# auniquesun/PPT

Measured on AMD Instinct MI355X. Metric: point-clouds/sec fwd+bwd, PointBERT 1024-pt ModelNet40, higher is better.
Workload: dtype f16; 1 GPU; C2: ModelNet40 1024-pt PointBERT (ULIP_PointBERT head_type=0, frozen backbone + PromptLearner), train-mode BN + DropPath, fwd + CE(ls 0.2) + bwd + AdamW; feed=resident, per_gpu_batch=32, global_batch=32, npoints=1024, classes=40, parallelism=dp1

## Files before the change

### ppt_amd/csrc/attention.hip

```cpp
#include "attn_common.h"

namespace {

constexpr int SEG = 16, KT = 32, ROWS = 64;

__device__ __forceinline__ float quad_sum(float v)
{
    v += __uint_as_float(dpp_mov<0xB1, 0xf>(__float_as_uint(v)));
    v += __uint_as_float(dpp_mov<0x4E, 0xf>(__float_as_uint(v)));
    return v;
}

template <typename T>
__device__ __forceinline__ void stage_rows(const T *__restrict__ base, int64_t row_stride, int r0, int Tlen,
                                           float *dst, int Tfull, int P, int v)
{
    for (int i = threadIdx.x; i < KT * HD; i += blockDim.x) {
        const int r = i >> 6, d = i & 63;
        dst[i] = (r0 + r) < Tlen ? dt<T>::load(base + am_row(Tfull, P, v, r0 + r) * row_stride + d) : 0.0f;
    }
}

template <typename T>
__global__ __launch_bounds__(256) void attn_fwd_quad(const T *__restrict__ qkv, T *__restrict__ out,
// ... 167 lines not shown
        dk[d] = 0.f; dv[d] = 0.f;
    }
    const int nqt = (Tlen + KT - 1) / KT;
    const int qt0 = causal ? (blockIdx.x * ROWS) / KT : 0;
    for (int qt = qt0; qt < nqt; ++qt) {
        __syncthreads();
        stage_rows<T>(qb, rs, qt * KT, Tlen, Qs, Tfull, P, b);
        stage_rows<T>(gb, (int64_t)H * HD, qt * KT, Tlen, Gs, Tfull, P, b);
        if (threadIdx.x < KT) {
            const int qi = qt * KT + threadIdx.x;
            Ls[threadIdx.x] = qi < Tlen ? lse[am_stat(Tfull, P, H, b, h, qi)] : 0.f;
            Ds[threadIdx.x] = qi < Tlen ? delta[am_stat(Tfull, P, H, b, h, qi)] : 0.f;
        }
        __syncthreads();
#pragma unroll 4
        for (int i = 0; i < KT; ++i) {
            float s = 0.f, dp = 0.f;
#pragma unroll
            for (int d = 0; d < SEG; ++d) {
                s = fmaf(Qs[i * HD + seg * SEG + d], k[d], s);
                dp = fmaf(Gs[i * HD + seg * SEG + d], v[d], dp);
            }
            s = quad_sum(s) * scale;
            dp = quad_sum(dp);
            const int qi = qt * KT + i;
            const bool ok = active && qi < Tlen && qi >= q_lo && (!causal || kj <= qi);
            const float p = ok ? __expf(s - Ls[i]) : 0.f;
            const float ds = p * (dp - Ds[i]) * scale;
#pragma unroll
            for (int d = 0; d < SEG; ++d) {
                dv[d] = fmaf(p, Gs[i * HD + seg * SEG + d], dv[d]);
                dk[d] = fmaf(ds, Qs[i * HD + seg * SEG + d], dk[d]);
            }
        }
    }
    if (active && P > 0 && kj < P) {
        float *pk = part + (((int64_t)b * P + kj) * 2) * (H * HD) + h * HD + seg * SEG, *pv = pk + H * HD;
#pragma unroll
        for (int d = 0; d < SEG; ++d) { pk[d] = dk[d]; pv[d] = dv[d]; }
    } else if (active) {
        T *o = dqkv + am_row(Tfull, P, b, kj) * rs + h * HD + seg * SEG;
#pragma unroll
        for (int d = 0; d < SEG; ++d) {
            dt<T>::store(o + H * HD + d, dk[d]);
            dt<T>::store(o + 2 * H * HD + d, dv[d]);
        }
    }
}

template <typename T>
__global__ __launch_bounds__(256) void attn_prefix_reduce(const float *__restrict__ part, int nseq, int P, int HHD, T *__restrict__ dqkv, int prio)
{
    PPT_PRIO(prio);
    const int i = blockIdx.x * 256 + threadIdx.x;
    if (i >= P * 2 * HHD) return;
    float acc = 0.f;
    const float *src = part + i;
    const int64_t stride = (int64_t)P * 2 * HHD;
    int v = 0;
    for (; v + 8 <= nseq; v += 8) {
        float t[8];
#pragma unroll
        for (int u = 0; u < 8; ++u) t[u] = src[(v + u) * stride];
#pragma unroll
        for (int u = 0; u < 8; ++u) acc += t[u];
    }
    for (; v < nseq; ++v) acc += src[v * stride];
    const int pos = i / (2 * HHD), rem = i - pos * 2 * HHD;
    dt<T>::store(dqkv + (int64_t)pos * 3 * HHD + HHD + rem, acc);
}

template <typename T>
int attn_fwd_t(const void *qkv, void *out, float *lse, int Bt, int Tl, int H, float scale, int causal, int P, hipStream_t s)
{
    dim3 grid((Tl + ROWS - 1) / ROWS, (Bt + (P > 0)) * H);
    hipLaunchKernelGGL(attn_fwd_quad<T>, grid, dim3(256), 0, s, (const T *)qkv, (T *)out, lse, Tl, H, scale, causal, P, Bt);
    PPT_CHECK_LAUNCH();
    return PPT_OK;
}

__host__ int64_t attn_rows(int Bt, int Tl, int P) { return P > 0 ? (int64_t)P + (int64_t)Bt * (Tl - P) : (int64_t)Bt * Tl; }

template <typename T>
int attn_reduce_t(const float *part, void *dqkv, int Bt, int P, int H, int prio, hipStream_t s)
{
    if (P <= 0) return PPT_OK;
    const int n = P * 2 * H * HD;
    hipLaunchKernelGGL(attn_prefix_reduce<T>, dim3((n + 255) / 256), dim3(256), 0, s, part, Bt + 1, P, H * HD, (T *)dqkv, prio);
    PPT_CHECK_LAUNCH();
    return PPT_OK;
}

template <typename T>
int attn_bwd_t(const void *qkv, const void *out, const void *dout, const float *lse, float *delta, void *dqkv,
               int Bt, int Tl, int H, float scale, int causal, int P, float *part, bool with_delta, hipStream_t s)
{
    if (with_delta) {
        const int64_t rows = attn_rows(Bt, Tl, P) * H;
        hipLaunchKernelGGL(attn_delta<T>, dim3((unsigned)((rows + 63) / 64)), dim3(256), 0, s, (const T *)out,
                           (const T *)dout, delta, Tl, H, rows, P);
        PPT_CHECK_LAUNCH();
    }
    dim3 grid((Tl + ROWS - 1) / ROWS, (Bt + (P > 0)) * H);
    hipLaunchKernelGGL(attn_bwd_dq<T>, grid, dim3(256), 0, s, (const T *)qkv, (const T *)dout, lse, delta, (T *)dqkv,
                       Tl, H, scale, causal, P, Bt);
    PPT_CHECK_LAUNCH();
    hipLaunchKernelGGL(attn_bwd_dkv<T>, grid, dim3(256), 0, s, (const T *)qkv, (const T *)dout, lse, delta, (T *)dqkv,
                       Tl, H, scale, causal, P, Bt, part);
    PPT_CHECK_LAUNCH();
    return attn_reduce_t<T>(part, dqkv, Bt, P, H, ppt_get_wave_priority(), s);
}

}

static int attn_fwd_any(const void *qkv, void *out, float *lse, int Bt, int T, int P, int H, int hd, float scale, int causal,
                        int dtype, void *stream)
{
    if (!qkv || !out || Bt <= 0 || T <= 0 || H <= 0 || hd != HD) return PPT_EINVAL;
    if (dtype == PPT_F32) return attn_fwd_t<float>(qkv, out, lse, Bt, T, H, scale, causal, P, ppt_stream(stream));
    if (dtype == PPT_BF16 || dtype == PPT_F16) return ppt_attention_fwd_mfma_bf16(qkv, out, lse, Bt, T, H, scale, causal, P, dtype, ppt_stream(stream));
    return PPT_EINVAL;
}

extern "C" int ppt_attention_fwd(const void *qkv, void *out, float *lse, int Bt, int T, int H, int hd, float scale,
                                 int causal, int dtype, void *stream)
{
    return attn_fwd_any(qkv, out, lse, Bt, T, 0, H, hd, scale, causal, dtype, stream);
}

extern "C" int ppt_attention_fwd_quad_bf16(const void *qkv, void *out, float *lse, int Bt, int T, int H, float scale,
                                           int causal, int P, int fmt, hipStream_t s)
{
    return fmt == PPT_F16 ? attn_fwd_t<f16_t>(qkv, out, lse, Bt, T, H, scale, causal, P, s) : attn_fwd_t<bf16_t>(qkv, out, lse, Bt, T, H, scale, causal, P, s);
}

extern "C" int ppt_attention_prefix_reduce_f32(const float *part, void *dqkv, int Bt, int P, int H, int prio, hipStream_t s)
{
    return attn_reduce_t<float>(part, dqkv, Bt, P, H, prio, s);
}

static int attn_bwd_any(const void *qkv, const void *out, const void *dout, const float *lse, float *delta, void *dqkv, float *part,
                        int Bt, int T, int P, int H, int hd, float scale, int causal, int dtype, void *stream)
{
    if (!qkv || !out || !dout || !lse || !delta || !dqkv || Bt <= 0 || T <= 0 || H <= 0 || hd != HD) return PPT_EINVAL;
    if (P > 0 && !part) return PPT_EINVAL;
    if (dtype == PPT_F32)
        return attn_bwd_t<float>(qkv, out, dout, lse, delta, dqkv, Bt, T, H, scale, causal, P, part, true, ppt_stream(stream));
    if (dtype == PPT_BF16 || dtype == PPT_F16) {
        hipStream_t s = ppt_stream(stream);
        const bool f16 = dtype == PPT_F16;
        const int prio = ppt_get_wave_priority();
        auto reduce = [&]() { return f16 ? attn_reduce_t<f16_t>(part, dqkv, Bt, P, H, prio, s) : attn_reduce_t<bf16_t>(part, dqkv, Bt, P, H, prio, s); };
        if (T <= 128) {
            const int rc = ppt_attention_bwd_short_mfma_bf16(qkv, out, dout, lse, dqkv, Bt, T, H, scale, causal, P, part, dtype, s);
            if (rc == PPT_OK) return reduce();
            if (rc != PPT_EUNSUPPORTED) return rc;
        }
        const int64_t rows = attn_rows(Bt, T, P) * H;
        if (f16)
            hipLaunchKernelGGL(attn_delta<f16_t>, dim3((unsigned)((rows + 63) / 64)), dim3(256), 0, s, (const f16_t *)out,
                               (const f16_t *)dout, delta, T, H, rows, P);
        else
            hipLaunchKernelGGL(attn_delta<bf16_t>, dim3((unsigned)((rows + 63) / 64)), dim3(256), 0, s, (const bf16_t *)out,
                               (const bf16_t *)dout, delta, T, H, rows, P);
        PPT_CHECK_LAUNCH();
        const int rc = ppt_attention_bwd_mfma_bf16(qkv, dout, lse, delta, dqkv, Bt, T, H, scale, causal, P, part, dtype, s);
        if (rc == PPT_OK) return reduce();
        if (rc != PPT_EUNSUPPORTED) return rc;
        return f16 ? attn_bwd_t<f16_t>(qkv, out, dout, lse, delta, dqkv, Bt, T, H, scale, causal, P, part, false, s)
                   : attn_bwd_t<bf16_t>(qkv, out, dout, lse, delta, dqkv, Bt, T, H, scale, causal, P, part, false, s);
    }
    return PPT_EINVAL;
}

extern "C" int ppt_attention_bwd(const void *qkv, const void *out, const void *dout, const float *lse, float *delta,
                                 void *dqkv, int Bt, int T, int H, int hd, float scale, int causal, int dtype,
                                 void *stream)
{
    return attn_bwd_any(qkv, out, dout, lse, delta, dqkv, nullptr, Bt, T, 0, H, hd, scale, causal, dtype, stream);
}

extern "C" size_t ppt_attention_prefix_workspace_bytes(int C, int P, int H, int hd)
{
    return (size_t)(C + 1) * (size_t)P * 2 * (size_t)H * (size_t)hd * sizeof(float);
}

extern "C" int ppt_attention_prefix_fwd(const void *qkv, void *out, float *lse, int C, int T, int P, int H, int hd, float scale,
                                        int dtype, void *stream)
{
    if (P <= 0 || P >= T) return PPT_EINVAL;
    return attn_fwd_any(qkv, out, lse, C, T, P, H, hd, scale, 1, dtype, stream);
}

extern "C" int ppt_attention_prefix_bwd(const void *qkv, const void *out, const void *dout, const float *lse, float *delta,
                                        void *dqkv, float *part, int C, int T, int P, int H, int hd, float scale, int dtype,
                                        void *stream)
{
    if (P <= 0 || P >= T) return PPT_EINVAL;
    return attn_bwd_any(qkv, out, dout, lse, delta, dqkv, part, C, T, P, H, hd, scale, 1, dtype, stream);
}
```

### ppt_amd/csrc/attention_mfma.hip

```cpp
#include <stdlib.h>
#include <type_traits>
#include "attn_bwd16.h"

namespace {

template <int FORM> struct AttnForm {
    using F = typename std::conditional<FORM == PPT_BF16, bf16_t, f16_t>::type;
    using T = bf16_t;
    using chunk_t = uint4;
    static constexpr int IMAGES = 1, CH_SHIFT = 3;
    static constexpr float P_PRE = 1.0f;
    struct Q { chunk_t raw[4][1]; };

    static __device__ __forceinline__ chunk_t zero() { return make_uint4(0, 0, 0, 0); }
    static __device__ __forceinline__ void prep_q(Q &, int) {}
    static __device__ __forceinline__ void write(unsigned char *kimg, unsigned char *vimg, int row, int ch, const chunk_t &k, const chunk_t &v)
    {
        *reinterpret_cast<uint4 *>(kimg + k_off(row, ch)) = k;
        *reinterpret_cast<uint4 *>(vimg + v_off(row, ch * 16)) = v;
    }
    static __device__ __forceinline__ float peel_dot(const T *kl, const Q &q, int h)
    {
        float dot = 0.f;
#pragma unroll
// ... 648 lines not shown
            const float *DL = reinterpret_cast<const float *>(base + 4 * QTILE + 128);
            ATTN_BWD_DKV_STEP(base + 0 * QTILE, base + 1 * QTILE, base + 2 * QTILE, base + 3 * QTILE, L2, DL, 0, qt * QT);
        }
        if (qt + 1 < nqt) write_tile(cur ^ 1);
        __syncthreads();
    }
    if (key < T && P > 0 && key < P) {
        float *pk = part + (((int64_t)b * P + key) * 2) * os + head * HD;
        attn_store_dkdv_part(pk, pk + os, dkt, dvt, h);
    } else if (key < T) {
        bf16_t *ok = dqkv + am_row(Tfull, P, b, key) * rs + head * HD + H * HD;
        attn_store_dkdv16<F>(ok, ok + H * HD, dkt, dvt, h);
    }
}

template <bool CAUSAL, typename F>
__global__ __launch_bounds__(256, 2) void attn_bwd_dkv_mfma(const bf16_t *__restrict__ qkv, const bf16_t *__restrict__ dout,
                                                         const float *__restrict__ lse, const float *__restrict__ delta,
                                                         bf16_t *__restrict__ dqkv, int Tfull, int H, float scale, int P, int C,
                                                         float *__restrict__ part)
{
    __shared__ __align__(16) unsigned char smem[DKV_SMEM];
    attn_bwd_dkv_body<F, CAUSAL, false>(qkv, nullptr, dout, lse, delta, dqkv, Tfull, H, scale, P, C, part, smem, blockIdx.x, blockIdx.y);
}

constexpr int DQ_SMEM = 2 * 3 * TILE;

template <typename F, bool CAUSAL, bool INLINE_DELTA>
__device__ __forceinline__ void attn_bwd_dq_body(const bf16_t *__restrict__ qkv, const bf16_t *__restrict__ out, const bf16_t *__restrict__ dout,
                                                 const float *__restrict__ lse, const float *__restrict__ delta,
                                                 bf16_t *__restrict__ dqkv, int Tfull, int H, float scale, int P, int C,
                                                 unsigned char *smem, const int bx, const int by)
{
    const int lane = threadIdx.x & 63;
    const int w = __builtin_amdgcn_readfirstlane(threadIdx.x >> 6);
    const int r = lane & 31, h = lane >> 5;
    const int bh = by, b = bh / H, head = bh % H;
    const int64_t rs = 3 * (int64_t)H * HD, os = (int64_t)H * HD;
    const int T = am_len(Tfull, P, C, b), q_lo = am_qlo(P, C, b);
    const bf16_t *qb = qkv + head * HD;
    const bf16_t *kb = qb + H * HD, *vb = qb + 2 * H * HD;
    const bf16_t *gb = dout + head * HD;
    const int q0 = bx * QB + w * 32;
    const int qrow = q0 + r;
    const float c = scale * 1.4426950408889634f;

    uint4 qf[4], gf[4];
    float dsum = 0.f;
#pragma unroll
    for (int kk = 0; kk < 4; ++kk) {
        uint4 a = make_uint4(0, 0, 0, 0), v = make_uint4(0, 0, 0, 0);
        if (qrow < T) {
            a = *reinterpret_cast<const uint4 *>(qb + am_row(Tfull, P, b, qrow) * rs + 16 * kk + 8 * h);
            v = *reinterpret_cast<const uint4 *>(gb + am_row(Tfull, P, b, qrow) * os + 16 * kk + 8 * h);
            if constexpr (INLINE_DELTA)
                dsum += dot8_bf16<F>(v, *reinterpret_cast<const uint4 *>(out + head * HD + am_row(Tfull, P, b, qrow) * os + 16 * kk + 8 * h));
        }
        qf[kk] = (a);
        gf[kk] = (v);
    }
    const bool own = qrow < T && qrow >= q_lo;
    const float l2 = own ? lse[am_stat(Tfull, P, H, b, head, qrow)] * 1.4426950408889634f : INFINITY;
    float dl;
    if constexpr (INLINE_DELTA) {
        const float ds = xor32_sum(dsum);
        dl = own ? ds : 0.f;
    } else dl = own ? delta[am_stat(Tfull, P, H, b, head, qrow)] : 0.f;

    uint4 sk[2], sv[2];
    auto load_tile = [&](int kt) {
#pragma unroll
        for (int i = 0; i < 2; ++i) {
            const int cidx = threadIdx.x + 256 * i;
            const int kx = kt * KVT + (cidx >> 3), ch = cidx & 7;
            sk[i] = sv[i] = make_uint4(0, 0, 0, 0);
            if (kx < T) {
                const int64_t kr = am_row(Tfull, P, b, kx) * rs;
                sk[i] = *reinterpret_cast<const uint4 *>(kb + kr + ch * 8);
                sv[i] = *reinterpret_cast<const uint4 *>(vb + kr + ch * 8);
            }
        }
    };
    auto write_tile = [&](int buf) {
#pragma unroll
        for (int i = 0; i < 2; ++i) {
            const int cidx = threadIdx.x + 256 * i;
            const int row = cidx >> 3, ch = cidx & 7;
            unsigned char *base = smem + buf * 3 * TILE;
            *reinterpret_cast<uint4 *>(base + 0 * TILE + k_off(row, ch)) = sk[i];
            *reinterpret_cast<uint4 *>(base + 1 * TILE + v_off(row, ch * 16)) = sk[i];
            *reinterpret_cast<uint4 *>(base + 2 * TILE + k_off(row, ch)) = sv[i];
        }
    };
    const int q_hi = min(T, (int)(bx + 1) * QB) - 1;
    const int nkt = CAUSAL ? min((T + KVT - 1) / KVT, q_hi / KVT + 1) : (T + KVT - 1) / KVT;
    f32x16_t dqt[2];
    ATTN_ZERO2(dqt[0], dqt[1]);
    int tr_row, tr_dbyte;
    tr_lane(lane, tr_row, tr_dbyte);

    load_tile(0);
    write_tile(0);
    __syncthreads();
    for (int kt = 0; kt < nkt; ++kt) {
        const int cur = kt & 1;
        if (kt + 1 < nkt) load_tile(kt + 1);
        const bool active = q0 < T && (!CAUSAL || kt * KVT <= q0 + 31);
        if (active) {
            const unsigned char *base = smem + cur * 3 * TILE;
            const bool need_mask = (kt * KVT + KVT > T) || (CAUSAL && kt * KVT + KVT - 1 > q0);
#pragma unroll
            for (int sub = 0; sub < 2; ++sub)
                ATTN_BWD_DQ_STEP(base + 0 * TILE, base + 1 * TILE, base + 2 * TILE, 32 * sub, kt * KVT + 32 * sub, need_mask);
        }
        if (kt + 1 < nkt) write_tile(cur ^ 1);
        __syncthreads();
    }
    if (own) attn_store_dq16<F>(dqkv + am_row(Tfull, P, b, qrow) * rs + head * HD, dqt, h);
}

template <bool CAUSAL, typename F>
__global__ __launch_bounds__(256, 2) void attn_bwd_dq_mfma(const bf16_t *__restrict__ qkv, const bf16_t *__restrict__ dout,
                                                        const float *__restrict__ lse, const float *__restrict__ delta,
                                                        bf16_t *__restrict__ dqkv, int Tfull, int H, float scale, int P, int C)
{
    __shared__ __align__(16) unsigned char smem[DQ_SMEM];
    attn_bwd_dq_body<F, CAUSAL, false>(qkv, nullptr, dout, lse, delta, dqkv, Tfull, H, scale, P, C, smem, blockIdx.x, blockIdx.y);
}

#ifndef PPT_SHORT_OCC
#define PPT_SHORT_OCC 2
#endif
template <bool CAUSAL, typename F>
__global__ __launch_bounds__(256, PPT_SHORT_OCC) void attn_bwd_short_mfma(const bf16_t *__restrict__ qkv, const bf16_t *__restrict__ out,
                                                           const bf16_t *__restrict__ dout, const float *__restrict__ lse,
                                                           bf16_t *__restrict__ dqkv, int Tfull, int H, float scale, int P, int C,
                                                           float *__restrict__ part, int prio)
{
    PPT_PRIO(prio);
    __shared__ __align__(16) unsigned char smem[DQ_SMEM > DKV_SMEM ? DQ_SMEM : DKV_SMEM];
#ifdef PPT_SHORT_ROLE
    if (PPT_SHORT_ROLE == 0) { attn_bwd_dkv_body<F, CAUSAL, true>(qkv, out, dout, lse, nullptr, dqkv, Tfull, H, scale, P, C, part, smem, 0, blockIdx.y); return; }
    if (PPT_SHORT_ROLE == 1) { attn_bwd_dq_body<F, CAUSAL, true>(qkv, out, dout, lse, nullptr, dqkv, Tfull, H, scale, P, C, smem, 0, blockIdx.y); return; }
    if (PPT_SHORT_ROLE == 2) return;
#endif
    if (gridDim.x == 1 || blockIdx.x == 0)
        attn_bwd_dkv_body<F, CAUSAL, true>(qkv, out, dout, lse, nullptr, dqkv, Tfull, H, scale, P, C, part, smem, 0, blockIdx.y);
    if (gridDim.x == 1) __syncthreads();
    if (gridDim.x == 1 || blockIdx.x == 1)
        attn_bwd_dq_body<F, CAUSAL, true>(qkv, out, dout, lse, nullptr, dqkv, Tfull, H, scale, P, C, smem, 0, blockIdx.y);
}


constexpr int TINY_SMEM = 7 * TILE + 512;
template <bool CAUSAL, typename F>
__global__ __launch_bounds__(256, 2) void attn_bwd_tiny_mfma(const bf16_t *__restrict__ qkv, const bf16_t *__restrict__ out,
                                                          const bf16_t *__restrict__ dout, const float *__restrict__ lse,
                                                          bf16_t *__restrict__ dqkv, int Tfull, int H, float scale, int P, int C,
                                                          float *__restrict__ part, int prio)
{
    PPT_PRIO(prio);
    __shared__ __align__(16) unsigned char smem[TINY_SMEM];
    unsigned char *Qr = smem, *Qt = smem + TILE, *Gr = smem + 2 * TILE, *Gt = smem + 3 * TILE, *Kr = smem + 4 * TILE, *Kt = smem + 5 * TILE,
                  *Vr = smem + 6 * TILE;
    float *L2 = reinterpret_cast<float *>(smem + 7 * TILE), *DL = L2 + 64;
    const int lane = threadIdx.x & 63;
    const int w = __builtin_amdgcn_readfirstlane(threadIdx.x >> 6);
    const int r = lane & 31, h = lane >> 5;
    const int bh = blockIdx.y, b = bh / H, head = bh % H;
    const int64_t rs = 3 * (int64_t)H * HD, os = (int64_t)H * HD;
    const int T = am_len(Tfull, P, C, b), q_lo = am_qlo(P, C, b);
    const float c = scale * 1.4426950408889634f;

    {
        uint4 q[2], k[2], v[2], g[2];
        float dl[2], l2[2];
#pragma unroll
        for (int i = 0; i < 2; ++i) {
            const int row = 32 * i + (threadIdx.x >> 3), ch = threadIdx.x & 7;
            q[i] = k[i] = v[i] = g[i] = make_uint4(0, 0, 0, 0);
            uint4 o = make_uint4(0, 0, 0, 0);
            l2[i] = INFINITY;
            const bool own = row < T && row >= q_lo;
            if (row < T) {
                const int64_t pr = am_row(Tfull, P, b, row);
                const bf16_t *qp = qkv + pr * rs + head * HD + ch * 8;
                q[i] = *reinterpret_cast<const uint4 *>(qp);
                k[i] = *reinterpret_cast<const uint4 *>(qp + H * HD);
                v[i] = *reinterpret_cast<const uint4 *>(qp + 2 * H * HD);
                g[i] = *reinterpret_cast<const uint4 *>(dout + pr * os + head * HD + ch * 8);
                o = *reinterpret_cast<const uint4 *>(out + pr * os + head * HD + ch * 8);
                if (own && ch == 0) l2[i] = lse[am_stat(Tfull, P, H, b, head, row)] * 1.4426950408889634f;
            }
            float d = dot8_bf16<F>(g[i], o);
            d += __shfl_xor(d, 1); d += __shfl_xor(d, 2); d += __shfl_xor(d, 4);
            dl[i] = own ? d : 0.f;
        }
#pragma unroll
        for (int i = 0; i < 2; ++i) {
            const int row = 32 * i + (threadIdx.x >> 3), ch = threadIdx.x & 7;
            *reinterpret_cast<uint4 *>(Qr + k_off(row, ch)) = q[i];
            *reinterpret_cast<uint4 *>(Qt + v_off(row, ch * 16)) = q[i];
            *reinterpret_cast<uint4 *>(Gr + k_off(row, ch)) = g[i];
            *reinterpret_cast<uint4 *>(Gt + v_off(row, ch * 16)) = g[i];
            *reinterpret_cast<uint4 *>(Kr + k_off(row, ch)) = k[i];
            *reinterpret_cast<uint4 *>(Kt + v_off(row, ch * 16)) = k[i];
            *reinterpret_cast<uint4 *>(Vr + k_off(row, ch)) = v[i];
            if (ch == 0) { L2[row] = l2[i]; DL[row] = dl[i]; }
        }
    }
    __syncthreads();
    int tr_row, tr_dbyte;
    tr_lane(lane, tr_row, tr_dbyte);

    if (w < 2) {
        const int k0 = 32 * w, key = k0 + r;
        if (k0 >= T) return;
        uint4 kf[4], vf[4];
#pragma unroll
        for (int kk = 0; kk < 4; ++kk) {
            kf[kk] = *reinterpret_cast<const uint4 *>(Kr + k_off(key, 2 * kk + h));
            vf[kk] = *reinterpret_cast<const uint4 *>(Vr + k_off(key, 2 * kk + h));
        }
        f32x16_t dvt[2], dkt[2];
#pragma unroll
    for (int i = 0; i < 2; ++i) ATTN_ZERO2(dvt[i], dkt[i]);
        const int nqt = (T + QT - 1) / QT;
        for (int qt = q_lo / QT; qt < nqt; ++qt) {
            if (CAUSAL && qt * QT + QT - 1 < k0) continue;
            ATTN_BWD_DKV_STEP(Qr, Qt, Gr, Gt, L2, DL, QT * qt, qt * QT);
        }
        if (key < T && P > 0 && key < P) {
            float *pk = part + (((int64_t)b * P + key) * 2) * os + head * HD;
            attn_store_dkdv_part(pk, pk + os, dkt, dvt, h);
        } else if (key < T) {
            bf16_t *ok = dqkv + am_row(Tfull, P, b, key) * rs + head * HD + H * HD;
            attn_store_dkdv16<F>(ok, ok + H * HD, dkt, dvt, h);
        }
    } else {
        const int q0 = 32 * (w - 2), qrow = q0 + r;
        if (q0 >= T || q0 + 31 < q_lo) return;
        uint4 qf[4], gf[4];
#pragma unroll
        for (int kk = 0; kk < 4; ++kk) {
            qf[kk] = *reinterpret_cast<const uint4 *>(Qr + k_off(qrow, 2 * kk + h));
            gf[kk] = *reinterpret_cast<const uint4 *>(Gr + k_off(qrow, 2 * kk + h));
        }
        const bool own = qrow < T && qrow >= q_lo;
        const float l2 = L2[qrow], dl = DL[qrow];
        f32x16_t dqt[2];
    ATTN_ZERO2(dqt[0], dqt[1]);
#pragma unroll
        for (int sub = 0; sub < 2; ++sub) {
            if (32 * sub >= T || (CAUSAL && 32 * sub > q0 + 31)) continue;
            ATTN_BWD_DQ_STEP(Kr, Kt, Vr, 32 * sub, 32 * sub, true);
        }
        if (own) attn_store_dq16<F>(dqkv + am_row(Tfull, P, b, qrow) * rs + head * HD, dqt, h);
    }
}

}

template <int FORM>
static int launch_fwd_stream(const void *qkv, void *out, float *lse, int Bt, int T, int H, float scale, int causal, int P, hipStream_t s)
{
    using E = typename AttnForm<FORM>::T;
    static const int xcd_map = getenv("PPT_ATTN_XCD_MAP") == nullptr || atoi(getenv("PPT_ATTN_XCD_MAP")) != 0;
    const float c = scale * 1.4426950408889634f;
    const int prio = ppt_get_wave_priority();
    const dim3 grid((T + QB - 1) / QB, (Bt + (P > 0)) * H), block(256);
    if (causal) hipLaunchKernelGGL((attn_fwd_stream<FORM, true>), grid, block, 0, s, (const E *)qkv, (E *)out, lse, T, H, c, P, Bt, prio, xcd_map);
    else hipLaunchKernelGGL((attn_fwd_stream<FORM, false>), grid, block, 0, s, (const E *)qkv, (E *)out, lse, T, H, c, P, Bt, prio, xcd_map);
    PPT_CHECK_LAUNCH();
    return PPT_OK;
}

extern "C" int ppt_attention_fwd_stream(const void *qkv, void *out, float *lse, int Bt, int T, int H, float scale, int causal, int P,
                                        int form, hipStream_t s)
{
    if (form == PPT_F32) return launch_fwd_stream<PPT_F32>(qkv, out, lse, Bt, T, H, scale, causal, P, s);
    if (form == PPT_F16) return launch_fwd_stream<PPT_F16>(qkv, out, lse, Bt, T, H, scale, causal, P, s);
    return launch_fwd_stream<PPT_BF16>(qkv, out, lse, Bt, T, H, scale, causal, P, s);
}

extern "C" int ppt_attention_fwd_mfma_bf16(const void *qkv, void *out, float *lse, int Bt, int T, int H, float scale,
                                           int causal, int P, int fmt, hipStream_t s)
{
    if (((uintptr_t)qkv & 15) || ((uintptr_t)out & 7)) return ppt_attention_fwd_quad_bf16(qkv, out, lse, Bt, T, H, scale, causal, P, fmt, s);
    const float c = scale * 1.4426950408889634f;
    const int prio = ppt_get_wave_priority();
    static const bool resident_ok = getenv("PPT_ATTN_RESIDENT") == nullptr || atoi(getenv("PPT_ATTN_RESIDENT")) != 0;
    if (resident_ok && !causal && P == 0 && (T % KVT) == 1 && T - 1 >= 6 * KVT && T - 1 <= RES_MAXK && Bt * H >= 128) {
        PPT_RAISE_LDS_ONCE(RES_LDS, (const void *)attn_fwd_resident<bf16_t, 6>, (const void *)attn_fwd_resident<bf16_t, 7>,
                           (const void *)attn_fwd_resident<bf16_t, 8>, (const void *)attn_fwd_resident<f16_t, 6>,
                           (const void *)attn_fwd_resident<f16_t, 7>, (const void *)attn_fwd_resident<f16_t, 8>);
        const int n = (T - 1) / KVT;
        ppt_launch16(fmt, [&](auto f) {
            using F = decltype(f);
            const auto k = n == 6 ? attn_fwd_resident<F, 6> : n == 7 ? attn_fwd_resident<F, 7> : attn_fwd_resident<F, 8>;
            hipLaunchKernelGGL(k, dim3(Bt * H), dim3(512), RES_LDS, s, (const bf16_t *)qkv, (bf16_t *)out, lse, T, H, c, prio);
        });
        PPT_CHECK_LAUNCH();
        return PPT_OK;
    }
    return ppt_attention_fwd_stream(qkv, out, lse, Bt, T, H, scale, causal, P, fmt, s);
}

extern "C" int ppt_attention_bwd_short_mfma_bf16(const void *qkv, const void *out, const void *dout, const float *lse, void *dqkv, int Bt, int T,
                                                 int H, float scale, int causal, int P, float *part, int fmt, hipStream_t s)
{
    if (T > 128) return PPT_EUNSUPPORTED;
    if (((uintptr_t)qkv & 15) || ((uintptr_t)out & 15) || ((uintptr_t)dout & 15) || ((uintptr_t)dqkv & 7) || ((uintptr_t)part & 15)) return PPT_EUNSUPPORTED;
    static const int both = [] { const char *e = getenv("PPT_ATTN_SHORT_BOTH"); return e ? atoi(e) : 1; }();
    static const int tiny = [] { const char *e = getenv("PPT_ATTN_TINY"); return e ? atoi(e) : 1; }();
    const int pairs = (Bt + (P > 0)) * H;
    if (tiny && T <= 64 && !((uintptr_t)dout & 15)) {
        const int prio = ppt_get_wave_priority();
        ppt_launch16(fmt, [&](auto f) {
            using F = decltype(f);
            const auto k = causal ? attn_bwd_tiny_mfma<true, F> : attn_bwd_tiny_mfma<false, F>;
            hipLaunchKernelGGL(k, dim3(1, pairs), dim3(256), 0, s, (const bf16_t *)qkv, (const bf16_t *)out, (const bf16_t *)dout, lse,
                               (bf16_t *)dqkv, T, H, scale, P, Bt, part, prio);
        });
        PPT_CHECK_LAUNCH();
        return PPT_OK;
    }
    dim3 grid(both && 2 * pairs > 512 ? 1 : 2, pairs);
    const int prio = ppt_get_wave_priority();
    ppt_launch16(fmt, [&](auto f) {
        using F = decltype(f);
        const auto k = causal ? attn_bwd_short_mfma<true, F> : attn_bwd_short_mfma<false, F>;
        hipLaunchKernelGGL(k, grid, dim3(256), 0, s, (const bf16_t *)qkv, (const bf16_t *)out, (const bf16_t *)dout, lse, (bf16_t *)dqkv, T, H,
                           scale, P, Bt, part, prio);
    });
    PPT_CHECK_LAUNCH();
    return PPT_OK;
}

extern "C" int ppt_attention_bwd_mfma_bf16(const void *qkv, const void *dout, const float *lse, const float *delta,
                                           void *dqkv, int Bt, int T, int H, float scale, int causal, int P, float *part,
                                           int fmt, hipStream_t s)
{
    if (((uintptr_t)qkv & 15) || ((uintptr_t)dout & 15) || ((uintptr_t)dqkv & 7) || ((uintptr_t)part & 15)) return PPT_EUNSUPPORTED;
    dim3 grid((T + 127) / 128, (Bt + (P > 0)) * H);
    ppt_launch16(fmt, [&](auto f) {
        using F = decltype(f);
        const auto dkv = causal ? attn_bwd_dkv_mfma<true, F> : attn_bwd_dkv_mfma<false, F>;
        const auto dq = causal ? attn_bwd_dq_mfma<true, F> : attn_bwd_dq_mfma<false, F>;
        hipLaunchKernelGGL(dkv, grid, dim3(256), 0, s, (const bf16_t *)qkv, (const bf16_t *)dout, lse, delta, (bf16_t *)dqkv, T, H, scale, P, Bt, part);
        hipLaunchKernelGGL(dq, grid, dim3(256), 0, s, (const bf16_t *)qkv, (const bf16_t *)dout, lse, delta, (bf16_t *)dqkv, T, H, scale, P, Bt);
    });
    PPT_CHECK_LAUNCH();
    return PPT_OK;
}
```

### ppt_amd/csrc/attn_common.h

```cpp
#pragma once
#include "ppt_common.h"
#include "attn_rowmap.h"

typedef __attribute__((ext_vector_type(4))) short s4_t;
typedef __attribute__((ext_vector_type(16))) float f32x16_t;

constexpr int HD = 64, KVT = 64, QB = 128, TILE = KVT * 128;
constexpr int QT = 32, QTILE = QT * 128;

__device__ __forceinline__ int k_off(int row, int chunk) { return row * 128 + ((chunk ^ ((row >> 1) & 7)) << 4); }
__device__ __forceinline__ int v_off(int key, int dbyte) { return key * 128 + (dbyte ^ (((key >> 1) & 1) << 6)); }

__device__ __forceinline__ uint4 tr_frag(const unsigned char *img, int row0, int dbyte)
{
    struct { s4_t a, b; } f;
    f.a = __builtin_amdgcn_ds_read_tr16_b64_v4i16((__attribute__((address_space(3))) s4_t *)(img + v_off(row0, dbyte)));
    f.b = __builtin_amdgcn_ds_read_tr16_b64_v4i16((__attribute__((address_space(3))) s4_t *)(img + v_off(row0 + 8, dbyte)));
    return __builtin_bit_cast(uint4, f);
}
__device__ __forceinline__ void tr_lane(int lane, int &tr_row, int &tr_dbyte)
{
    const int g = lane >> 4, tq = (lane >> 2) & 3, tp = lane & 3;
    tr_row = 4 * (g >> 1) + tq;
    tr_dbyte = (16 * (g & 1) + 4 * tp) * 2;
}

#define ATTN_ZERO2(a, b)                                                                            \
    do {                                                                                            \
        _Pragma("unroll") for (int e_ = 0; e_ < 16; ++e_) { (a)[e_] = 0.f; (b)[e_] = 0.f; }         \
    } while (0)

__device__ __forceinline__ void attn_xcd_map(int xcd_map, int &qblk, int &bh)
{
    bh = blockIdx.y, qblk = blockIdx.x;
    if (xcd_map && (gridDim.y & 7) == 0) {
        const int lin = blockIdx.y * gridDim.x + blockIdx.x, slot = lin >> 3;
        bh = (slot / (int)gridDim.x) * 8 + (lin & 7);
        qblk = slot % (int)gridDim.x;
    }
}

template <typename F>
__device__ __forceinline__ uint4 pack8(const f32x16_t &x, int s)
{
    return make_uint4(h16<F>::pack2(x[8 * s + 0], x[8 * s + 1]), h16<F>::pack2(x[8 * s + 2], x[8 * s + 3]),
                      h16<F>::pack2(x[8 * s + 4], x[8 * s + 5]), h16<F>::pack2(x[8 * s + 6], x[8 * s + 7]));
}

typedef _Float16 h2_t __attribute__((ext_vector_type(2)));

__device__ __forceinline__ void split2(float a, float b, uint32_t &hi, uint32_t &lo)
{
    const _Float16 ha = (_Float16)a, hb = (_Float16)b;
    const h2_t hh = {ha, hb};
    const h2_t ll = {(_Float16)(a - (float)ha), (_Float16)(b - (float)hb)};
    hi = __builtin_bit_cast(uint32_t, hh);
    lo = __builtin_bit_cast(uint32_t, ll);
}
__device__ __forceinline__ void split8(const float4 &u, const float4 &v, uint4 &hi, uint4 &lo)
{
    split2(u.x, u.y, hi.x, lo.x); split2(u.z, u.w, hi.y, lo.y);
    split2(v.x, v.y, hi.z, lo.z); split2(v.z, v.w, hi.w, lo.w);
}
__device__ __forceinline__ f32x16_t mfma3(uint4 ah, uint4 al, uint4 bh, uint4 bl, f32x16_t c)
{
    c = h16<f16_t>::mfma32(al, bh, c);
    c = h16<f16_t>::mfma32(ah, bl, c);
    return h16<f16_t>::mfma32(ah, bh, c);
}
__device__ __forceinline__ void split_acc(const f32x16_t &x, int s, uint4 &hi, uint4 &lo)
{
    split2(x[8 * s + 0], x[8 * s + 1], hi.x, lo.x); split2(x[8 * s + 2], x[8 * s + 3], hi.y, lo.y);
    split2(x[8 * s + 4], x[8 * s + 5], hi.z, lo.z); split2(x[8 * s + 6], x[8 * s + 7], hi.w, lo.w);
}

extern "C" {
int ppt_attention_fwd_stream(const void *qkv, void *out, float *lse, int Bt, int T, int H, float scale, int causal, int P, int form,
                             hipStream_t s);
int ppt_attention_fwd_mfma_bf16(const void *qkv, void *out, float *lse, int Bt, int T, int H, float scale, int causal, int P, int fmt,
                                hipStream_t s);
int ppt_attention_bwd_mfma_bf16(const void *qkv, const void *dout, const float *lse, const float *delta, void *dqkv, int Bt, int T,
                                int H, float scale, int causal, int P, float *part, int fmt, hipStream_t s);
int ppt_attention_bwd_short_mfma_bf16(const void *qkv, const void *out, const void *dout, const float *lse, void *dqkv, int Bt, int T,
                                      int H, float scale, int causal, int P, float *part, int fmt, hipStream_t s);
int ppt_attention_fwd_quad_bf16(const void *qkv, void *out, float *lse, int Bt, int T, int H, float scale, int causal, int P, int fmt,
                                hipStream_t s);
int ppt_attention_prefix_reduce_f32(const float *part, void *dqkv, int Bt, int P, int H, int prio, hipStream_t s);
}
```

Measured before the change: 11730 point-clouds/s.

## Fold shared-prefix dK/dV reduction into tiny attention backward kernel

The tiny attention backward kernel now gets extra owner blocks, one per head, that stream every batch row's Q, dO, O and LSE through LDS in 128-row stages. They accumulate the dK/dV for the shared prompt-prefix keys directly and write them to dqkv. This replaces the per-sequence partial-sum buffer and the separate prefix-reduce kernel launch, removing its memory traffic and launch cost. The price is a serialized loop in the owner blocks over all batch rows, a larger dynamic LDS allocation that may hurt occupancy, and a cross-wave fold through shared memory.

```diff
diff --git a/ppt_amd/csrc/attention.hip b/ppt_amd/csrc/attention.hip
--- a/ppt_amd/csrc/attention.hip
+++ b/ppt_amd/csrc/attention.hip
@@ -343,8 +343,9 @@
         const int prio = ppt_get_wave_priority();
         auto reduce = [&]() { return f16 ? attn_reduce_t<f16_t>(part, dqkv, Bt, P, H, prio, s) : attn_reduce_t<bf16_t>(part, dqkv, Bt, P, H, prio, s); };
         if (T <= 128) {
-            const int rc = ppt_attention_bwd_short_mfma_bf16(qkv, out, dout, lse, dqkv, Bt, T, H, scale, causal, P, part, dtype, s);
-            if (rc == PPT_OK) return reduce();
+            int folded = 0;
+            const int rc = ppt_attention_bwd_short_mfma_bf16(qkv, out, dout, lse, dqkv, Bt, T, H, scale, causal, P, part, dtype, s, &folded);
+            if (rc == PPT_OK) return folded ? PPT_OK : reduce();
             if (rc != PPT_EUNSUPPORTED) return rc;
         }
         const int64_t rows = attn_rows(Bt, T, P) * H;
diff --git a/ppt_amd/csrc/attention_mfma.hip b/ppt_amd/csrc/attention_mfma.hip
--- a/ppt_amd/csrc/attention_mfma.hip
+++ b/ppt_amd/csrc/attention_mfma.hip
@@ -824,25 +824,60 @@
 }
 
 
-constexpr int TINY_SMEM = 7 * TILE + 512;
+constexpr int OWN_ROWS = 128;
+constexpr int OWN_IMG = OWN_ROWS * 128;
+constexpr int TINY_SMEM = 4 * OWN_IMG + 2 * OWN_ROWS * 4;
+static_assert(TINY_SMEM >= 7 * TILE + 512, "the seven 64-row images + lse2[64] + delta[64] of the staged (sequence, head)");
+static_assert(4 * OWN_IMG >= 3 * 64 * 64 * 4, "three waves' accumulators for the fold");
+
 template <bool CAUSAL, typename F>
 __global__ __launch_bounds__(256, 2) void attn_bwd_tiny_mfma(const bf16_t *__restrict__ qkv, const bf16_t *__restrict__ out,
                                                           const bf16_t *__restrict__ dout, const float *__restrict__ lse,
-                                                          bf16_t *__restrict__ dqkv, int Tfull, int H, float scale, int P, int C,
-                                                          float *__restrict__ part, int prio)
+                                                          bf16_t *__restrict__ dqkv, int Tfull, int H, float scale, int P, int C, int prio)
 {
     PPT_PRIO(prio);
-    __shared__ __align__(16) unsigned char smem[TINY_SMEM];
+    extern __shared__ __align__(16) unsigned char smem[];
     unsigned char *Qr = smem, *Qt = smem + TILE, *Gr = smem + 2 * TILE, *Gt = smem + 3 * TILE, *Kr = smem + 4 * TILE, *Kt = smem + 5 * TILE,
                   *Vr = smem + 6 * TILE;
     float *L2 = reinterpret_cast<float *>(smem + 7 * TILE), *DL = L2 + 64;
     const int lane = threadIdx.x & 63;
     const int w = __builtin_amdgcn_readfirstlane(threadIdx.x >> 6);
     const int r = lane & 31, h = lane >> 5;
-    const int bh = blockIdx.y, b = bh / H, head = bh % H;
+    const int bh = blockIdx.y, b = P > 0 ? (bh < H ? C : bh / H - 1) : bh / H, head = bh % H;
     const int64_t rs = 3 * (int64_t)H * HD, os = (int64_t)H * HD;
     const int T = am_len(Tfull, P, C, b), q_lo = am_qlo(P, C, b);
     const float c = scale * 1.4426950408889634f;
+    const bool owner = CAUSAL && P > 0 && b == C;
+
+    const int R = C * (Tfull - P), nst = (R + OWN_ROWS - 1) / OWN_ROWS;
+    uint4 own_q[4], own_g[4], own_o[4];
+    float own_l2;
+    auto own_load = [&](int st) {
+#pragma unroll
+        for (int j = 0; j < 4; ++j) {
+            const int64_t pr = P + min(st * OWN_ROWS + 32 * j + (int)(threadIdx.x >> 3), R - 1);
+            const uint4 q = *reinterpret_cast<const uint4 *>(qkv + pr * rs + head * HD + (threadIdx.x & 7) * 8);
+            own_q[j] = make_uint4(q.x, q.y, q.z, q.w);
+            own_g[j] = *reinterpret_cast<const uint4 *>(dout + pr * os + head * HD + (threadIdx.x & 7) * 8);
+            own_o[j] = *reinterpret_cast<const uint4 *>(out + pr * os + head * HD + (threadIdx.x & 7) * 8);
+        }
+        own_l2 = lse[((int64_t)P + min(st * OWN_ROWS + (int)(threadIdx.x & (OWN_ROWS - 1)), R - 1)) * H + head];
+    };
+    auto own_write = [&](int st) {
+        float *SL2 = reinterpret_cast<float *>(smem + 4 * OWN_IMG), *SDL = SL2 + OWN_ROWS;
+#pragma unroll
+        for (int j = 0; j < 4; ++j) {
+            const int row = 32 * j + (threadIdx.x >> 3), ch = threadIdx.x & 7;
+            *reinterpret_cast<uint4 *>(smem + 0 * OWN_IMG + k_off(row, ch)) = own_q[j];
+            *reinterpret_cast<uint4 *>(smem + 1 * OWN_IMG + v_off(row, ch * 16)) = own_q[j];
+            *reinterpret_cast<uint4 *>(smem + 2 * OWN_IMG + k_off(row, ch)) = own_g[j];
+            *reinterpret_cast<uint4 *>(smem + 3 * OWN_IMG + v_off(row, ch * 16)) = own_g[j];
+            float d = dot8_bf16<F>(own_g[j], own_o[j]);
+            d += __shfl_xor(d, 1); d += __shfl_xor(d, 2); d += __shfl_xor(d, 4);
+            if (ch == 0) SDL[row] = d;
+        }
+        if (threadIdx.x < OWN_ROWS) SL2[threadIdx.x] = st * OWN_ROWS + (int)threadIdx.x < R ? own_l2 * 1.4426950408889634f : INFINITY;
+    };
 
     {
         uint4 q[2], k[2], v[2], g[2];
@@ -868,6 +903,7 @@
             d += __shfl_xor(d, 1); d += __shfl_xor(d, 2); d += __shfl_xor(d, 4);
             dl[i] = own ? d : 0.f;
         }
+        if (owner) own_load(0);
 #pragma unroll
         for (int i = 0; i < 2; ++i) {
             const int row = 32 * i + (threadIdx.x >> 3), ch = threadIdx.x & 7;
@@ -885,49 +921,101 @@
     int tr_row, tr_dbyte;
     tr_lane(lane, tr_row, tr_dbyte);
 
+    uint4 kf[4], vf[4];
+    f32x16_t dvt[2], dkt[2];
     if (w < 2) {
         const int k0 = 32 * w, key = k0 + r;
-        if (k0 >= T) return;
-        uint4 kf[4], vf[4];
-#pragma unroll
-        for (int kk = 0; kk < 4; ++kk) {
-            kf[kk] = *reinterpret_cast<const uint4 *>(Kr + k_off(key, 2 * kk + h));
-            vf[kk] = *reinterpret_cast<const uint4 *>(Vr + k_off(key, 2 * kk + h));
-        }
-        f32x16_t dvt[2], dkt[2];
-#pragma unroll
-    for (int i = 0; i < 2; ++i) ATTN_ZERO2(dvt[i], dkt[i]);
-        const int nqt = (T + QT - 1) / QT;
-        for (int qt = q_lo / QT; qt < nqt; ++qt) {
-            if (CAUSAL && qt * QT + QT - 1 < k0) continue;
-            ATTN_BWD_DKV_STEP(Qr, Qt, Gr, Gt, L2, DL, QT * qt, qt * QT);
-        }
-        if (key < T && P > 0 && key < P) {
-            float *pk = part + (((int64_t)b * P + key) * 2) * os + head * HD;
-            attn_store_dkdv_part(pk, pk + os, dkt, dvt, h);
-        } else if (key < T) {
-            bf16_t *ok = dqkv + am_row(Tfull, P, b, key) * rs + head * HD + H * HD;
-            attn_store_dkdv16<F>(ok, ok + H * HD, dkt, dvt, h);
+#pragma unroll
+        for (int i = 0; i < 2; ++i) ATTN_ZERO2(dvt[i], dkt[i]);
+        const bool live = k0 < T && (owner || k0 + 32 > P);
+        if (live) {
+#pragma unroll
+            for (int kk = 0; kk < 4; ++kk) {
+                kf[kk] = *reinterpret_cast<const uint4 *>(Kr + k_off(key, 2 * kk + h));
+                vf[kk] = *reinterpret_cast<const uint4 *>(Vr + k_off(key, 2 * kk + h));
+            }
+            const int nqt = (T + QT - 1) / QT;
+            for (int qt = q_lo / QT; qt < nqt; ++qt) {
+                if (CAUSAL && qt * QT + QT - 1 < k0) continue;
+                ATTN_BWD_DKV_STEP(Qr, Qt, Gr, Gt, L2, DL, QT * qt, qt * QT);
+            }
+        }
+        if (!owner) {
+            if (live && key < T && key >= P) {
+                bf16_t *ok = dqkv + am_row(Tfull, P, b, key) * rs + head * HD + H * HD;
+                attn_store_dkdv16<F>(ok, ok + H * HD, dkt, dvt, h);
+            }
+            return;
         }
     } else {
         const int q0 = 32 * (w - 2), qrow = q0 + r;
-        if (q0 >= T || q0 + 31 < q_lo) return;
-        uint4 qf[4], gf[4];
-#pragma unroll
-        for (int kk = 0; kk < 4; ++kk) {
-            qf[kk] = *reinterpret_cast<const uint4 *>(Qr + k_off(qrow, 2 * kk + h));
-            gf[kk] = *reinterpret_cast<const uint4 *>(Gr + k_off(qrow, 2 * kk + h));
-        }
-        const bool own = qrow < T && qrow >= q_lo;
-        const float l2 = L2[qrow], dl = DL[qrow];
-        f32x16_t dqt[2];
-    ATTN_ZERO2(dqt[0], dqt[1]);
-#pragma unroll
-        for (int sub = 0; sub < 2; ++sub) {
-            if (32 * sub >= T || (CAUSAL && 32 * sub > q0 + 31)) continue;
-            ATTN_BWD_DQ_STEP(Kr, Kt, Vr, 32 * sub, 32 * sub, true);
-        }
-        if (own) attn_store_dq16<F>(dqkv + am_row(Tfull, P, b, qrow) * rs + head * HD, dqt, h);
+        if (q0 < T && q0 + 31 >= q_lo) {
+            uint4 qf[4], gf[4];
+#pragma unroll
+            for (int kk = 0; kk < 4; ++kk) {
+                qf[kk] = *reinterpret_cast<const uint4 *>(Qr + k_off(qrow, 2 * kk + h));
+                gf[kk] = *reinterpret_cast<const uint4 *>(Gr + k_off(qrow, 2 * kk + h));
+            }
+            const bool own = qrow < T && qrow >= q_lo;
+            const float l2 = L2[qrow], dl = DL[qrow];
+            f32x16_t dqt[2];
+            ATTN_ZERO2(dqt[0], dqt[1]);
+#pragma unroll
+            for (int sub = 0; sub < 2; ++sub) {
+                if (32 * sub >= T || (CAUSAL && 32 * sub > q0 + 31)) continue;
+                ATTN_BWD_DQ_STEP(Kr, Kt, Vr, 32 * sub, 32 * sub, true);
+            }
+            if (own) attn_store_dq16<F>(dqkv + am_row(Tfull, P, b, qrow) * rs + head * HD, dqt, h);
+        }
+        if (!owner) return;
+#pragma unroll
+        for (int i = 0; i < 2; ++i) ATTN_ZERO2(dvt[i], dkt[i]);
+    }
+
+    const int nkh = P > 32 ? 2 : 1, nqg = 4 / nkh;
+    const int kh = nkh == 2 ? (w & 1) : 0, qg = nkh == 2 ? (w >> 1) : w;
+    const int k0 = 32 * kh, key = k0 + r;
+#pragma unroll
+    for (int kk = 0; kk < 4; ++kk) {
+        kf[kk] = *reinterpret_cast<const uint4 *>(Kr + k_off(key, 2 * kk + h));
+        vf[kk] = *reinterpret_cast<const uint4 *>(Vr + k_off(key, 2 * kk + h));
+    }
+    __syncthreads();
+    for (int st = 0; st < nst; ++st) {
+        own_write(st);
+        if (st + 1 < nst) own_load(st + 1);
+        __syncthreads();
+        const float *SL2 = reinterpret_cast<const float *>(smem + 4 * OWN_IMG), *SDL = SL2 + OWN_ROWS;
+        for (int t = qg; t < OWN_ROWS / QT; t += nqg)
+            if (st * OWN_ROWS + QT * t < R)
+                ATTN_BWD_DKV_STEP(smem, smem + OWN_IMG, smem + 2 * OWN_IMG, smem + 3 * OWN_IMG, SL2, SDL, QT * t, KVT);
+        __syncthreads();
+    }
+    float4 *slab = reinterpret_cast<float4 *>(smem);
+    if (w >= nkh) {
+#pragma unroll
+        for (int i = 0; i < 2; ++i)
+#pragma unroll
+            for (int e = 0; e < 4; ++e) {
+                slab[(((w - nkh) * 4 + i) * 4 + e) * 64 + lane] = make_float4(dkt[i][4 * e], dkt[i][4 * e + 1], dkt[i][4 * e + 2], dkt[i][4 * e + 3]);
+                slab[(((w - nkh) * 4 + 2 + i) * 4 + e) * 64 + lane] = make_float4(dvt[i][4 * e], dvt[i][4 * e + 1], dvt[i][4 * e + 2], dvt[i][4 * e + 3]);
+            }
+    }
+    __syncthreads();
+    if (w >= nkh) return;
+    for (int o = w; o < 4 - nkh; o += nkh) {
+#pragma unroll
+        for (int i = 0; i < 2; ++i)
+#pragma unroll
+            for (int e = 0; e < 4; ++e) {
+                const float4 a = slab[((o * 4 + i) * 4 + e) * 64 + lane], v = slab[((o * 4 + 2 + i) * 4 + e) * 64 + lane];
+                dkt[i][4 * e] += a.x; dkt[i][4 * e + 1] += a.y; dkt[i][4 * e + 2] += a.z; dkt[i][4 * e + 3] += a.w;
+                dvt[i][4 * e] += v.x; dvt[i][4 * e + 1] += v.y; dvt[i][4 * e + 2] += v.z; dvt[i][4 * e + 3] += v.w;
+            }
+    }
+    if (key < P) {
+        bf16_t *ok = dqkv + (int64_t)key * rs + head * HD + H * HD;
+        attn_store_dkdv16<F>(ok, ok + H * HD, dkt, dvt, h);
     }
 }
 
@@ -979,22 +1067,26 @@
 }
 
 extern "C" int ppt_attention_bwd_short_mfma_bf16(const void *qkv, const void *out, const void *dout, const float *lse, void *dqkv, int Bt, int T,
-                                                 int H, float scale, int causal, int P, float *part, int fmt, hipStream_t s)
-{
+                                                 int H, float scale, int causal, int P, float *part, int fmt, hipStream_t s, int *folded)
+{
+    *folded = 0;
     if (T > 128) return PPT_EUNSUPPORTED;
     if (((uintptr_t)qkv & 15) || ((uintptr_t)out & 15) || ((uintptr_t)dout & 15) || ((uintptr_t)dqkv & 7) || ((uintptr_t)part & 15)) return PPT_EUNSUPPORTED;
     static const int both = [] { const char *e = getenv("PPT_ATTN_SHORT_BOTH"); return e ? atoi(e) : 1; }();
     static const int tiny = [] { const char *e = getenv("PPT_ATTN_TINY"); return e ? atoi(e) : 1; }();
     const int pairs = (Bt + (P > 0)) * H;
-    if (tiny && T <= 64 && !((uintptr_t)dout & 15)) {
+    if (tiny && T <= 64 && (P == 0 || causal) && !((uintptr_t)dout & 15)) {
+        PPT_RAISE_LDS_ONCE(TINY_SMEM, (const void *)attn_bwd_tiny_mfma<true, bf16_t>, (const void *)attn_bwd_tiny_mfma<false, bf16_t>,
+                           (const void *)attn_bwd_tiny_mfma<true, f16_t>, (const void *)attn_bwd_tiny_mfma<false, f16_t>);
         const int prio = ppt_get_wave_priority();
         ppt_launch16(fmt, [&](auto f) {
             using F = decltype(f);
             const auto k = causal ? attn_bwd_tiny_mfma<true, F> : attn_bwd_tiny_mfma<false, F>;
-            hipLaunchKernelGGL(k, dim3(1, pairs), dim3(256), 0, s, (const bf16_t *)qkv, (const bf16_t *)out, (const bf16_t *)dout, lse,
-                               (bf16_t *)dqkv, T, H, scale, P, Bt, part, prio);
+            hipLaunchKernelGGL(k, dim3(1, pairs), dim3(256), TINY_SMEM, s, (const bf16_t *)qkv, (const bf16_t *)out, (const bf16_t *)dout, lse,
+                               (bf16_t *)dqkv, T, H, scale, P, Bt, prio);
         });
         PPT_CHECK_LAUNCH();
+        *folded = 1;
         return PPT_OK;
     }
     dim3 grid(both && 2 * pairs > 512 ? 1 : 2, pairs);
diff --git a/ppt_amd/csrc/attn_common.h b/ppt_amd/csrc/attn_common.h
--- a/ppt_amd/csrc/attn_common.h
+++ b/ppt_amd/csrc/attn_common.h
@@ -82,7 +82,7 @@
 int ppt_attention_bwd_mfma_bf16(const void *qkv, const void *dout, const float *lse, const float *delta, void *dqkv, int Bt, int T,
                                 int H, float scale, int causal, int P, float *part, int fmt, hipStream_t s);
 int ppt_attention_bwd_short_mfma_bf16(const void *qkv, const void *out, const void *dout, const float *lse, void *dqkv, int Bt, int T,
-                                      int H, float scale, int causal, int P, float *part, int fmt, hipStream_t s);
+                                      int H, float scale, int causal, int P, float *part, int fmt, hipStream_t s, int *folded);
 int ppt_attention_fwd_quad_bf16(const void *qkv, void *out, float *lse, int Bt, int T, int H, float scale, int causal, int P, int fmt,
                                 hipStream_t s);
 int ppt_attention_prefix_reduce_f32(const float *part, void *dqkv, int Bt, int P, int H, int prio, hipStream_t s);
```

Measured after the change: 11700 point-clouds/s. No clear change (-0.2%).
